# nmonette/TO-UED

Hardware: NVIDIA B200
Metric: gridworld agent env-steps/sec incl. LPG update (higher is better)
Workload: dtype f16/bf16 operands, f32 accumulate (GRU); f32 elsewhere

## Files before the change

include/toued.h:

```cpp
#ifndef TOUED_H
#define TOUED_H
#include <stdint.h>
#ifdef __cplusplus
extern "C" {
#endif

#define TOUED_LEVEL_BYTES 192

const char* toued_last_error(void);
int toued_version(void);

int toued_rollout(const void* levels, const uint32_t* keys, const float* actor,
                  const uint8_t* forced_actions, int32_t* state, int32_t* obs, uint8_t* action,
                  float* reward, uint8_t* done, float* ep_return, int n_agents, int n_workers,
                  int rollout_len, int obs_dim, int max_grid_size, int max_n_objs, int reset_first,
                  void* stream);

int toued_env_step(const void* levels, const uint32_t* keys, const int32_t* actions, int32_t* state,
                   int32_t* obs, float* reward, uint8_t* done, int n_agents, int n_workers,
                   int max_grid_size, int max_n_objs, void* stream);
int toued_env_reset(const void* levels, int32_t* state, int32_t* obs, int n_agents, int n_workers,
                    int max_grid_size, void* stream);


// ... 78 lines not shown
                    float lr_actor, float lr_critic, float max_grad_norm, float gamma, float gae_lambda,
                    float entropy_coeff, int outer_product_quirk, void* stream);

int toued_es_ask(const uint32_t* key, const float* mean, float sigma, float* candidates, int popsize,
                 int n_params, int cand_stride, void* stream);
int toued_es_tell(const float* candidates, const float* fitness, float* mean, float* m, float* v,
                  int popsize, int n_params, int cand_stride, float sigma, float lrate, float beta1,
                  float beta2, float eps, int gen_counter, float mean_decay, void* stream);

int toued_es_ask_shard(const uint32_t* key, const float* mean, float sigma, float* candidates, int popsize_global,
                       int n_params, int cand_stride, int pair_offset, int n_pairs, void* stream);
int toued_es_grad_partial(const float* candidates, const float* fitness, const float* mean, float* grad_sum,
                          int n_members, int n_params, int cand_stride, float sigma, void* stream);
int toued_es_adam(const float* grad_sum, float* mean, float* m, float* v, int popsize_global, int n_params,
                  float sigma, float lrate, float beta1, float beta2, float eps, int gen_counter, float mean_decay,
                  void* stream);

int toued_plr_reset_lowest(float* score, uint8_t* active, uint8_t* is_new, int buffer_size, int minimum_new,
                           int* reset_ids, void* stream);
int toued_plr_select(uint32_t key0, uint32_t key1, float* score, uint8_t* active, uint8_t* is_new, int buffer_size,
                     const int* old_ids, const uint8_t* terminated, const float* new_scores, int n_agents,
                     float p_replay, float temperature, int shuffle_rounds, int* new_ids, void* stream);

int toued_generate_levels_desc_bytes(void);
int toued_generate_levels(const void* gen_desc, const uint32_t* keys, const int32_t* buffer_ids, void* levels_out,
                          int32_t* lifetimes_out, int n_levels, void* stream);

int toued_optimal_return(const void* levels, int n_levels, int horizon, int max_grid_size, int max_n_objs,
                         double* out, void* stream);

int toued_get_nash(const float* game, const float* x0, const float* y0, float* x_out, float* y_out,
                   int n, int x_nz, int y_nz, int num_iters, float lr, void* stream);
int toued_projection_simplex(float* v, int n, int max_nz, void* stream);


int toued_init_tables(const uint32_t* keys, const uint8_t* mask, float* tables, int n_agents,
                      int obs_dim, int n_out, void* stream);
int toued_masked_reset(const void* levels, const uint8_t* mask, int32_t* state, int32_t* obs,
                       int32_t* step, int n_agents, int n_workers, int max_grid_size, void* stream);

int toued_host_iota_bits(const uint32_t* keys, int n_keys, int n, uint32_t* out);


int toued_key_split(const uint32_t* keys_in, int n_keys, int num, int offset, int count, uint32_t* out,
                    void* stream);
int toued_key_chain(const uint32_t* keys_in, int n_keys, int chain_len, uint32_t* keys_out,
                    uint32_t* carry_out, void* stream);


int toued_tc_gemm_test(const float* A, const float* B, void* scratch_img, float* D, void* stream);
int toued_tc_gemm_mixed_test(const float* A, const float* B, void* scratch_img, float* D, void* stream);
int toued_tc_gemm_mn_test(const float* A, const float* B, void* scratch_img, float* D, int lbo, int sbo,
                          int kadv, void* stream);
int toued_tc_gemm_mn2_test(const float* A, const float* B, void* scratch_img, float* D, void* stream);

int toued_pack_wh_forward(const float* lpg_params, void* wh_img, int lifetime_conditioning, void* stream);
int toued_gru_forward_tc(const float* x, const uint8_t* done, const float* lpg_params, const void* wh_img,
                         void* h16, void* fac, void* hpimg, float* pi_hat, float* y_hat, int n_agents,
                         int n_workers, int rollout_len, int lifetime_conditioning, void* stream);
int toued_pack_wh_forward_multi(const float* lpg_params, void* wh_img, int lifetime_conditioning, int n_sets,
                                int lpg_stride, void* stream);
int toued_gru_forward_tc_multi(const float* x, const uint8_t* done, const float* lpg_params, const void* wh_img,
                               float* pi_hat, float* y_hat, int n_agents, int n_workers, int rollout_len,
                               int lifetime_conditioning, int lpg_stride, void* stream);

int toued_pack_wh_backward(const float* lpg_params, void* whb_img, void* stream);
#define TOUED_STATUS_NONFINITE_COT 1u
#define TOUED_STATUS_FP16_RANGE 2u
int toued_cotangent_max(const float* d_pi_hat, const float* d_y_hat, int n_agents, int n_workers, int rollout_len,
                        uint32_t* cotangent_max, void* stream);
int toued_gru_backward_tc(const uint8_t* done, const float* lpg_params, const void* whb_img,
                          const void* h16, const void* fac, const float* y_hat, const float* d_pi_hat,
                          const float* d_y_hat, void* dgimg, float* dl, float* dx, uint32_t* cotangent_max,
                          int n_agents, int n_workers, int rollout_len, int lifetime_conditioning, void* stream);
int toued_wgrad_tc_splits(void);
int toued_wgrad_tc_small_splits(void);
int toued_lpg_wgrad_tc(const void* hpimg, const void* dgimg, const void* ximg, const void* h16,
                       const float* d_pi_hat, const float* dl, float* wh_partials, float* small_partials,
                       uint32_t* cotangent_max, int n_agents, int n_workers, int rollout_len, int accumulate,
                       void* stream);

#ifdef __cplusplus
}
#endif
#endif
```

to_ued_b200/_lib.py:

```python
from __future__ import annotations

import ctypes as C
import os

_HERE = os.path.dirname(os.path.abspath(__file__))
_VARIANT = os.environ.get("TOUED_LIB_VARIANT", "")
LIB_PATH = os.path.join(_HERE, f"libtoued_{_VARIANT}.so" if _VARIANT else "libtoued.so")

_lib = None


class TouedError(RuntimeError):
    pass


def lib() -> C.CDLL:
    global _lib
    if _lib is None:
        if not os.path.exists(LIB_PATH):
            raise TouedError(
                f"{LIB_PATH} is missing: the CUDA extension is not built. "
                "Run `python -m to_ued_b200.csrc.build` (there is no CPU fallback).")
        _lib = C.CDLL(LIB_PATH)
        _declare(_lib)
    return _lib


_P, _I, _F = C.c_void_p, C.c_int, C.c_float

SIGNATURES = {
    "toued_rollout": [_P] * 10 + [_I] * 7 + [_P],
    "toued_env_step": [_P] * 7 + [_I] * 4 + [_P],
    "toued_env_reset": [_P] * 3 + [_I] * 3 + [_P],
    "toued_sort_tokens": [_P] * 2 + [_I] * 3 + [_P],
    "toued_lpg_prepare": [_P] * 11 + [_I] * 6 + [_P],
    "toued_gru_forward": [_P] * 7 + [_I] * 5 + [_P],
    "toued_agent_update": [_P] * 12 + [_I] * 4 + [_F] * 4 + [_I, _P, _P],
    "toued_agent_scratch_floats": [_I] * 4,
    "toued_meta_loss": [_P] * 10 + [_I] * 5 + [_F] * 3 + [_I, _P],
    "toued_agent_backward": [_P] * 14 + [_I] * 4 + [_F] * 9 + [_P, _P],
    "toued_transpose_wh": [_P] * 3,
    "toued_gru_backward": [_P] * 10 + [_I] * 4 + [_P],
    "toued_lpg_wgrad_workspace_floats": [],
    "toued_lpg_wgrad": [_P] * 11 + [_I] * 6 + [_P],
    "toued_reduce_partials": [_P, _P, _I, _I, _I, _P],
    "toued_lpg_wgrad_splits": [_I],
    "toued_lpg_wgrad_workspace_offset": [_I],
    "toued_lpg_wgrad_embed": [_P] * 7 + [_I] * 6 + [_P],
    "toued_cotangent_max": [_P, _P, _I, _I, _I, _P, _P],
    "toued_pack_wh_backward": [_P] * 3,
    "toued_gru_backward_tc": [_P] * 12 + [_I] * 4 + [_P],
    "toued_wgrad_tc_splits": [],
    "toued_wgrad_tc_small_splits": [],
    "toued_lpg_wgrad_tc": [_P] * 9 + [_I] * 4 + [_P],
    "toued_adam": [_P] * 4 + [_I, _I] + [_F] * 4 + [_P],
    "toued_adam_dev": [_P] * 5 + [_I] + [_F] * 4 + [_P],
    "toued_sgd_clip": [_P] * 3 + [_I, _F, _F, _P],
    "toued_get_nash": [_P] * 5 + [_I] * 4 + [_F, _P],
    "toued_projection_simplex": [_P, _I, _I, _P],
    "toued_es_ask": [_P, _P, _F, _P, _I, _I, _I, _P],
    "toued_es_tell": [_P] * 5 + [_I, _I, _I] + [_F] * 5 + [_I, _F, _P],
    "toued_es_ask_shard": [_P, _P, _F, _P, _I, _I, _I, _I, _I, _P],
    "toued_es_grad_partial": [_P] * 4 + [_I, _I, _I, _F, _P],
    "toued_es_adam": [_P] * 4 + [_I, _I] + [_F] * 5 + [_I, _F, _P],
    "toued_a2c_update": [_P] * 12 + [_I] * 4 + [_F] * 6 + [_I, _P],
    "toued_a2c_train": [_P] * 15 + [_I] * 7 + [_F] * 6 + [_I, _P],
    "toued_init_tables": [_P] * 3 + [_I] * 3 + [_P],
    "toued_masked_reset": [_P] * 5 + [_I] * 3 + [_P],
    "toued_generate_levels_desc_bytes": [],
    "toued_generate_levels": [_P] * 5 + [_I, _P],
    "toued_plr_reset_lowest": [_P] * 3 + [_I, _I, _P, _P],
    "toued_plr_select": [C.c_uint32, C.c_uint32] + [_P] * 3 + [_I] + [_P] * 3 + [_I, _F, _F, _I, _P, _P],
    "toued_tc_gemm_test": [_P] * 5,
    "toued_tc_gemm_mixed_test": [_P] * 5,
    "toued_tc_gemm_mn_test": [_P] * 4 + [_I] * 3 + [_P],
    "toued_tc_gemm_mn2_test": [_P] * 5,
    "toued_pack_wh_forward": [_P, _P, _I, _P],
    "toued_pack_wh_forward_multi": [_P, _P, _I, _I, _I, _P],
    "toued_gru_forward_tc_multi": [_P] * 6 + [_I] * 5 + [_P],
    "toued_host_iota_bits": [_P, _I, _I, _P],
    "toued_key_split": [_P, _I, _I, _I, _I, _P, _P],
    "toued_key_chain": [_P, _I, _I, _P, _P, _P],
    "toued_gru_forward_tc": [_P] * 9 + [_I] * 4 + [_P],
    "toued_optimal_return": [_P] + [_I] * 4 + [_P, _P],
}


def _declare(l):
    l.toued_last_error.restype = C.c_char_p
    l.toued_last_error.argtypes = []
    l.toued_version.restype = _I
    l.toued_version.argtypes = []
    for name, args in SIGNATURES.items():
        fn = getattr(l, name)
        fn.restype = _I
        fn.argtypes = args


def ptr(t):
    if t is None:
        return None
    if not t.is_cuda:
        raise TouedError("to_ued_b200 ops need CUDA tensors (there is no CPU fallback)")
    if not t.is_contiguous():
        raise TouedError("to_ued_b200 ops need contiguous tensors")
    return t.data_ptr()


def stream_ptr():
    import torch
    return torch.cuda.current_stream().cuda_stream


KERNELS_PER_CALL = {"toued_adam_dev": 2, "toued_sgd_clip": 2, "toued_lpg_wgrad": 3, "toued_init_tables": 2, "toued_lpg_wgrad_tc": 2, "toued_pack_wh_forward": 2, "toued_pack_wh_forward_multi": 2}
LAUNCHES = {}
GRAPH_KERNELS = [0]
ENV_STEPS = [0]
PROFILE = None


H2D_BYTES = [0]


def h2d(t):
    H2D_BYTES[0] += int(t.numel() * t.element_size()) if hasattr(t, "element_size") else int(t.nbytes)
    return t


def reset_counters(profile=False):
# ... 34 lines not shown
```

to_ued_b200/csrc/gru_backward_tc.cu:

```cuda
#include "tc.cuh"
#include "lpg_common.cuh"
#include "../../include/toued.h"

constexpr int BT_M = 128;
constexpr int BT_THREADS = 11 * 32;
constexpr int BT_ACHUNK = BT_M * 128;
constexpr int BT_SSTAGE = 4 * BT_ACHUNK;
constexpr int BT_CSTAGE = 2 * BT_ACHUNK;
constexpr int BT_BSLICE = LPG_H * 32;
constexpr int BT_NSB = 6;
constexpr int BT_ICHUNK = 512;

__global__ void pack_wh_bwd_kernel(const float* __restrict__ Wh, __half* __restrict__ img) {
    const int i = blockIdx.x * blockDim.x + threadIdx.x;
    if (i >= LPG_H * LPG_G) return;
    const int j = i / LPG_G, c = i % LPG_G;
    char* base = reinterpret_cast<char*>(img) + (size_t)(c >> 4) * BT_BSLICE;
    *reinterpret_cast<__half*>(base + k16_offset(j, c & 15)) = __float2half_rn(Wh[i]);
}

extern "C" int toued_pack_wh_backward(const float* lpg_params, void* whb_img, void* stream) {
    pack_wh_bwd_kernel<<<(LPG_H * LPG_G + 255) / 256, 256, 0, (cudaStream_t)stream>>>(
        lpg_params + lpg_offsets(5).Wh, (__half*)whb_img);
    TOUED_LAUNCH_CHECK();
    return 0;
}

__device__ __forceinline__ uint4 ldg_stream(const __half* p) {
    uint4 r;
    asm volatile("ld.global.nc.L1::no_allocate.v4.u32 {%0, %1, %2, %3}, [%4];" : "=r"(r.x), "=r"(r.y), "=r"(r.z), "=r"(r.w) : "l"(p));
    return r;
}
__device__ __forceinline__ void unpack8h(const uint4& r, float (&v)[8]) {
    const __half2* h = reinterpret_cast<const __half2*>(&r);
#pragma unroll
    for (int e = 0; e < 4; ++e) { const float2 f = __half22float2(h[e]); v[2 * e] = f.x; v[2 * e + 1] = f.y; }
}
__global__ void __launch_bounds__(BT_THREADS, 1)
gru_backward_tc_kernel(const uint8_t* __restrict__ done, const float* __restrict__ lpg, int X,
                       const unsigned char* __restrict__ whb_img, const __half* __restrict__ h16,
                       const __half* __restrict__ fac, const float* __restrict__ y_hat,
                       const float* __restrict__ d_pi_hat, const float* __restrict__ d_y_hat,
                       unsigned char* __restrict__ dgimg, float* __restrict__ dl_out, float* __restrict__ dx,
                       uint32_t* __restrict__ cotmax, int R, int L, int W) {
    extern __shared__ __align__(1024) unsigned char smem_raw[];
    unsigned char* smem = smem_raw + ((1024u - (smem_u32(smem_raw) & 1023u)) & 1023u);
    unsigned char* sS = smem;
    unsigned char* sC = sS + 2 * BT_SSTAGE;
    unsigned char* sB = sC + BT_CSTAGE;
    unsigned char* sI = sB + BT_NSB * BT_BSLICE;
    float* swp = reinterpret_cast<float*>(sI + BT_ICHUNK);
    float* sWy = swp + LPG_H;
    float* sWi = sWy + LPG_H * LPG_Y;
    float* sWi2 = sWi + LPG_H * 4;
    float* sdx = sWi2 + LPG_H * 2;
    __shared__ __align__(8) uint64_t b_full[BT_NSB], b_empty[BT_NSB], k_full[4], k_empty[4], s_empty[2], q_full;
    __shared__ uint32_t tmem_base_s;

    const LpgOffsets o = lpg_offsets(X);
    const int tid = threadIdx.x, warp = tid >> 5, lane = tid & 31;
    const int row0 = blockIdx.x * BT_M;

    if (tid == 0) {
        for (int s = 0; s < BT_NSB; ++s) { mbar_init(&b_full[s], 1); mbar_init(&b_empty[s], 1); }
        for (int k = 0; k < 4; ++k) { mbar_init(&k_full[k], 4); mbar_init(&k_empty[k], 2); }
        mbar_init(&s_empty[0], 1); mbar_init(&s_empty[1], 1); mbar_init(&q_full, 1);
        mbar_fence_init();
    }
    if (warp == 9) tmem_alloc(&tmem_base_s, 512);
    for (int i = tid; i < LPG_H; i += BT_THREADS) swp[i] = lpg[o.w_pi + i];
    for (int i = tid; i < LPG_H * LPG_Y; i += BT_THREADS) sWy[i] = lpg[o.W_y + i];
    for (int i = tid; i < LPG_H * 6; i += BT_THREADS) {
        const int u = i / 6, q = i % 6;
        const float w = lpg[o.Wi + (3 + q / 3) * LPG_G + (q % 3) * LPG_H + u];
        if (q < 4) sWi[u * 4 + q] = w; else sWi2[u * 2 + q - 4] = w;
    }
    for (int i = tid; i < 16 * 16; i += BT_THREADS) {
        const int n = i >> 4, k = i & 15;
        *reinterpret_cast<__half*>(sI + k16_offset(n, k)) = __float2half_rn(n == k ? 1.0f : 0.0f);
    }
    fence_proxy_async_smem();
    tc_fence_before();
    __syncthreads();
    tc_fence_after();
    const uint32_t tmem_base = tmem_base_s;
    const size_t R32 = ((size_t)R + 31) >> 5;
    const size_t tstride = R32 * 32 * LPG_H;

    if (warp == 8) {
        if (lane == 0) {
            uint32_t it = 0;
            for (int t = 0; t < L; ++t) {
                if (t + 1 == L) break;
                for (int ub = 0; ub < 4; ++ub)
                    for (int kk = 0; kk < 4; ++kk) {
                        const int ks = ((kk & 1) << 1) | (kk >> 1);
                        for (int g = 0; g < 3; ++g, ++it) {
                            const int s = it % BT_NSB;
                            mbar_wait(&b_empty[s], ((it / BT_NSB) & 1) ^ 1);
                            mbar_expect_tx(&b_full[s], BT_BSLICE);
                            bulk_g2s(sB + s * BT_BSLICE, whb_img + (size_t)(g * 16 + ub * 4 + ks) * BT_BSLICE, BT_BSLICE, &b_full[s]);
                        }
                    }
            }
        }
    } else if (warp == 9) {
        {
            constexpr uint32_t idesc256 = tc_idesc(BT_M, 256, 0), idesc16 = tc_idesc(BT_M, 16, 0);
            const uint32_t s_addr = smem_u32(sS), c_addr = smem_u32(sC), i_addr = smem_u32(sI);
            const uint64_t cd0 = tc_smem_desc(c_addr), idd = tc_smem_desc_k16(i_addr);
            uint32_t it = 0;
            uint32_t ait = 0;
            for (int t = 0; t < L; ++t) {
                const uint32_t q_addr = tmem_base + (t & 1) * 256;
                const bool mma = t + 1 < L;
                for (int ub = 0; ub < 4; ++ub, ++ait) {
                    const uint64_t ad0 = tc_smem_desc(s_addr + (ait & 1) * BT_SSTAGE);
#pragma unroll
                    for (int kk = 0; kk < 4; ++kk) {
                        const int ks = ((kk & 1) << 1) | (kk >> 1);
                        uint32_t sg[3];
                        if (mma) {
#pragma unroll
                            for (int g = 0; g < 3; ++g, ++it) {
                                sg[g] = it % BT_NSB;
                                mbar_wait(&b_full[sg[g]], (it / BT_NSB) & 1);
                            }
                        }
                        mbar_wait(&k_full[ks], ait & 1);
                        tc_fence_after();
                        if (elect_one()) {
                            if (mma) {
#pragma unroll
                                for (int g = 0; g < 3; ++g)
                                    tc_mma(q_addr, ad0 + (uint64_t)((g * BT_ACHUNK) >> 4) + 2 * ks,
                                           tc_smem_desc_k16(smem_u32(sB + sg[g] * BT_BSLICE)), idesc256, (ub | kk | g) != 0);
                                tc_mma(q_addr + ub * 64 + ks * 16, cd0 + 2 * ks, idd, idesc16, 1u);
                                tc_mma(q_addr + ub * 64 + ks * 16, cd0 + (uint64_t)(BT_ACHUNK >> 4) + 2 * ks, idd, idesc16, 1u);
#pragma unroll
                                for (int g = 0; g < 3; ++g) tc_commit(&b_empty[sg[g]]);
                            }
                            tc_commit(&k_empty[ks]);
                            if (mma && ub == 3 && kk == 3) tc_commit(&q_full);
                        }
                        __syncwarp();
                    }
                }
            }
        }
    } else if (warp == 10) {
        if (lane == 0) {
            const uint32_t s_addr = smem_u32(sS);
            const size_t Rp = ((size_t)R + 63) & ~(size_t)63;
            const int nsub = ((size_t)row0 + 64 < Rp) ? 2 : 1;
            uint32_t ait = 0;
            for (int t = 0; t < L; ++t) {
                for (int ub = 0; ub < 4; ++ub, ++ait) {
#pragma unroll
                    for (int kk = 0; kk < 4; ++kk) {
                        const int ks = ((kk & 1) << 1) | (kk >> 1);
                        mbar_wait(&k_full[ks], ait & 1);
                        mbar_arrive(&k_empty[ks]);
                    }
                    const size_t itok0 = (size_t)t * Rp + row0;
                    const uint32_t src0 = s_addr + (ait & 1) * BT_SSTAGE;
#pragma unroll
                    for (int g = 0; g < 4; ++g)
                        for (int sub = 0; sub < nsub; ++sub)
                            bulk_s2g(dgimg + tile_img_offset(itok0 + sub * 64, 16, (g * 4 + ub) * 64), src0 + g * BT_ACHUNK + sub * 8192, 8192);
                    bulk_commit();
                    if (ait > 0) {
                        bulk_wait_read_1();
                        mbar_arrive(&s_empty[(ait - 1) & 1]);
                    }
                }
            }
            bulk_wait_read();
            mbar_arrive(&s_empty[(ait - 1) & 1]);
            bulk_wait_all();
        }
    } else {
        const int q = warp & 3, hf = warp >> 2;
        const int rl = q * 32 + lane;
        const int row = row0 + rl;
        const bool rv = row < R;
        const int rsafe = rv ? row : 0;
        const int n_ag = rsafe / W, w_ag = rsafe % W;
        uint32_t ait = 0;
        float range_max = 0.0f;
        const uint32_t sS_u32 = smem_u32(sS), sC_u32 = smem_u32(sC);
        const float S = cotmax ? cot_scale_from_max(*cotmax) : 1.0f;
        struct FacLoads { uint4 r, z, n, hn, hx; };
        const size_t fbase = rb32_index(0, R32, rsafe, hf * 32);
        const __half* p_r = fac + fac_index(0, R32, rsafe, hf * 32, 0);
        const __half* p_z = fac + fac_index(0, R32, rsafe, hf * 32, 1);
        const __half* p_n = fac + fac_index(0, R32, rsafe, hf * 32, 2);
        const __half* p_hn = fac + fac_index(0, R32, rsafe, hf * 32, 3);
        const __half* p_hx = h16 + fbase;
        const int tlast = L - 1;
        auto issue_fac = [&](int t_, int ub_, int c8_) {
            FacLoads l;
            const size_t off = (size_t)t_ * tstride + (size_t)((ub_ * 8 + c8_) << 8);
            const size_t foff = 4 * (size_t)t_ * tstride + (size_t)((ub_ * 8 + c8_) << 8);
            l.r = ldg_stream(p_r + foff);
            l.z = ldg_stream(p_z + foff);
            l.n = ldg_stream(p_n + foff);
            l.hn = ldg_stream(p_hn + foff);
            l.hx = ldg_stream(p_hx + off + (t_ < tlast ? tstride : 0));
            return l;
        };
        struct RowLoads { float4 y0, y1, d0, d1; float dpi; uint8_t dn, dn_hp; };
        auto issue_row = [&](int t_) {
            RowLoads r;
            const size_t tok_ = (size_t)t_ * R + rsafe;
            const float4* q0 = reinterpret_cast<const float4*>(y_hat + tok_ * 8);
            const float4* q1 = reinterpret_cast<const float4*>(d_y_hat + tok_ * 8);
            r.y0 = q0[0]; r.y1 = q0[1]; r.d0 = q1[0]; r.d1 = q1[1];
            r.dpi = d_pi_hat[tok_];
            r.dn = t_ > 0 ? done[((size_t)n_ag * L + (t_ - 1)) * W + w_ag] : (uint8_t)1;
            r.dn_hp = t_ + 1 < L ? done[((size_t)n_ag * L + t_) * W + w_ag] : (uint8_t)1;
            return r;
        };
        FacLoads nxt = issue_fac(0, 0, 0);
        RowLoads rnx = issue_row(0);
        for (int t = 0; t < L; ++t) {
            const size_t tok = (size_t)t * R + rsafe;
            float dl[8], dpi;
            const RowLoads rc = rnx;
            if (t + 1 < L) rnx = issue_row(t + 1);
            {
                const float yh[8] = {rc.y0.x, rc.y0.y, rc.y0.z, rc.y0.w, rc.y1.x, rc.y1.y, rc.y1.z, rc.y1.w};
                const float dy[8] = {rc.d0.x, rc.d0.y, rc.d0.z, rc.d0.w, rc.d1.x, rc.d1.y, rc.d1.z, rc.d1.w};
                float s = 0.f;
#pragma unroll
                for (int i = 0; i < 8; ++i) s = fmaf(yh[i], dy[i], s);
#pragma unroll
                for (int i = 0; i < 8; ++i) dl[i] = rv ? S * (yh[i] * (dy[i] - s)) : 0.0f;
                dpi = rv ? S * rc.dpi : 0.0f;
                if (hf == 0 && rv) {
                    float4* qo = reinterpret_cast<float4*>(dl_out + tok * 8);
                    qo[0] = make_float4(dl[0], dl[1], dl[2], dl[3]);
                    qo[1] = make_float4(dl[4], dl[5], dl[6], dl[7]);
                }
            }
            const float nd = (t > 0 && rv && !rc.dn) ? 1.0f : 0.0f;
            const float nd_hp = rc.dn_hp ? 0.0f : 1.0f;
            if (t > 0) { mbar_wait(&q_full, (t - 1) & 1); tc_fence_after(); }
            const uint32_t p_addr = tmem_base + ((t - 1) & 1) * 256 + ((uint32_t)(q * 32) << 16);
            float dx3 = 0.f, dx4 = 0.f;
            for (int ub = 0; ub < 4; ++ub) {
                const int ubase = ub * 64 + hf * 32;
                const uint32_t sSb = sS_u32 + (ait & 1) * BT_SSTAGE;
#pragma unroll
                for (int c8 = 0; c8 < 4; ++c8) {
                    const int u0 = ubase + c8 * 8;
                    float carry[8];
                    if (t > 0) tmem_ld8(p_addr + u0, carry);
                    const FacLoads cur = nxt;
                    {
                        int t2 = t, ub2 = ub, c2 = c8 + 1;
                        if (c2 == 4) { c2 = 0; ++ub2; if (ub2 == 4) { ub2 = 0; t2 = min(t + 1, tlast); } }
                        nxt = issue_fac(t2, ub2, c2);
                    }
                    if (t > 0) tmem_ld_wait();
                    else {
#pragma unroll
                        for (int e = 0; e < 8; ++e) carry[e] = 0.f;
                    }
                    float gr_[8], zz[8], gn_[8], hn_[8], hx[8];
                    const uint32_t zw[4] = {cur.z.x, cur.z.y, cur.z.z, cur.z.w};
                    unpack8h(cur.r, gr_); unpack8h(make_uint4(zw[0] & 0x7FFF7FFFu, zw[1] & 0x7FFF7FFFu, zw[2] & 0x7FFF7FFFu, zw[3] & 0x7FFF7FFFu), zz);
                    unpack8h(cur.n, gn_); unpack8h(cur.hn, hn_); unpack8h(cur.hx, hx);
                    float gr[8], gz[8], ghn[8], gan[8], cz[8];
#pragma unroll
                    for (int e = 0; e < 8; ++e) {
                        const int u = u0 + e;
                        float dh = nd * carry[e];
                        {
                            const float4 w0 = *reinterpret_cast<const float4*>(sWy + u * 8), w1 = *reinterpret_cast<const float4*>(sWy + u * 8 + 4);
                            float hd = dpi * swp[u];
                            hd = fmaf(dl[0], w0.x, hd); hd = fmaf(dl[1], w0.y, hd); hd = fmaf(dl[2], w0.z, hd); hd = fmaf(dl[3], w0.w, hd);
                            hd = fmaf(dl[4], w1.x, hd); hd = fmaf(dl[5], w1.y, hd); hd = fmaf(dl[6], w1.z, hd); hd = fmaf(dl[7], w1.w, hd);
                            dh += ((zw[e >> 1] >> (15 + 16 * (e & 1))) & 1u) ? 0.0f : hd;
                        }
                        if (!rv) dh = 0.0f;
                        const float omz = 1.0f - zz[e];
                        gan[e] = dh * omz * (1.0f - gn_[e] * gn_[e]);
                        ghn[e] = gan[e] * gr_[e];
                        gr[e] = ghn[e] * hn_[e] * (1.0f - gr_[e]);
                        gz[e] = dh * (nd_hp * hx[e] - gn_[e]) * zz[e] * omz;
                        cz[e] = dh * zz[e];
                        range_max = fmax3_nan(range_max, fabsf(dh), fabsf(gr[e]));
                        {
                            const float4 w0 = *reinterpret_cast<const float4*>(sWi + u * 4);
                            const float2 w1 = *reinterpret_cast<const float2*>(sWi2 + u * 2);
                            dx3 = fmaf(gr[e], w0.x, fmaf(gz[e], w0.y, fmaf(gan[e], w0.z, dx3)));
                            dx4 = fmaf(gr[e], w0.w, fmaf(gz[e], w1.x, fmaf(gan[e], w1.y, dx4)));
                        }
                    }
                    uint4 czh4, czl4;
                    {
                        uint32_t hi[4], lo[4];
#pragma unroll
                        for (int e2 = 0; e2 < 4; ++e2) {
                            hi[e2] = pack_h2_sat(cz[2 * e2], cz[2 * e2 + 1]);
                            const float2 f = __half22float2(*reinterpret_cast<const __half2*>(&hi[e2]));
                            lo[e2] = pack_h2_sat(cz[2 * e2] - f.x, cz[2 * e2 + 1] - f.y);
                        }
                        czh4 = make_uint4(hi[0], hi[1], hi[2], hi[3]);
                        czl4 = make_uint4(lo[0], lo[1], lo[2], lo[3]);
                    }
                    if (c8 == 0 && ait >= 2) mbar_wait(&s_empty[ait & 1], ((ait >> 1) & 1) ^ 1);
                    if ((c8 & 1) == 0 && ait > 0) mbar_wait(&k_empty[hf * 2 + (c8 >> 1)], (ait & 1) ^ 1);
                    const uint32_t so = sw128_offset(BT_M, rl, hf * 32 + c8 * 8);
                    st_shared_v4(sSb + so + 0 * BT_ACHUNK, pack8h_sat(gr));
                    st_shared_v4(sSb + so + 1 * BT_ACHUNK, pack8h_sat(gz));
                    st_shared_v4(sSb + so + 2 * BT_ACHUNK, pack8h_sat(ghn));
                    st_shared_v4(sSb + so + 3 * BT_ACHUNK, pack8h_sat(gan));
                    st_shared_v4(sC_u32 + so, czh4);
                    st_shared_v4(sC_u32 + so + BT_ACHUNK, czl4);
                    if (c8 & 1) {
                        fence_proxy_async_smem();
                        tc_fence_before();
                        __syncwarp();
                        if (lane == 0) mbar_arrive(&k_full[hf * 2 + (c8 >> 1)]);
                    }
                }
                ++ait;
            }
            if (hf > 0) { sdx[((hf - 1) * BT_M + rl) * 2] = dx3; sdx[((hf - 1) * BT_M + rl) * 2 + 1] = dx4; }
            asm volatile("bar.sync 1, 256;" ::: "memory");
            if (hf == 0 && rv) {
                dx3 += sdx[rl * 2]; dx4 += sdx[rl * 2 + 1];
                *reinterpret_cast<float2*>(dx + ((size_t)t * R + row) * 2) = make_float2(dx3, dx4);
            }
            asm volatile("bar.sync 1, 256;" ::: "memory");
        }
        if (__any_sync(0xffffffffu, !(range_max <= 65504.0f)) && lane == 0 && cotmax) atomicOr(cotmax + 1, TOUED_STATUS_FP16_RANGE);
    }
    tc_fence_before();
    __syncthreads();
    if (warp == 9) tmem_dealloc(tmem_base, 512);
}

static size_t gru_bwd_tc_smem() {
    return 2 * BT_SSTAGE + BT_CSTAGE + BT_NSB * BT_BSLICE + BT_ICHUNK + sizeof(float) * (LPG_H + LPG_H * LPG_Y + LPG_H * 6 + BT_M * 2) + 1024;
}

extern "C" int toued_gru_backward_tc(const uint8_t* done, const float* lpg_params, const void* whb_img,
                                     const void* h16, const void* fac, const float* y_hat, const float* d_pi_hat,
                                     const float* d_y_hat, void* dgimg, float* dl, float* dx, uint32_t* cotangent_max,
                                     int n_agents, int n_workers, int rollout_len, int lifetime_conditioning, void* stream) {
    const int R = n_agents * n_workers;
    TOUED_CHECK(R > 0 && rollout_len > 0, "toued_gru_backward_tc: empty problem");
    const size_t smem = gru_bwd_tc_smem();
    TOUED_CUDA(cudaFuncSetAttribute(gru_backward_tc_kernel, cudaFuncAttributeMaxDynamicSharedMemorySize, (int)smem));
    gru_backward_tc_kernel<<<(R + BT_M - 1) / BT_M, BT_THREADS, smem, (cudaStream_t)stream>>>(
        done, lpg_params, lifetime_conditioning ? 7 : 5, (const unsigned char*)whb_img, (const __half*)h16,
        (const __half*)fac, y_hat, d_pi_hat, d_y_hat, (unsigned char*)dgimg, dl, dx, cotangent_max, R, rollout_len, n_workers);
    TOUED_LAUNCH_CHECK();
    return 0;
}
```

to_ued_b200/csrc/tc.cuh:

```cuda
#pragma once
#include "common.cuh"
#include <cuda_fp16.h>
#include <cuda_bf16.h>

constexpr int TC_KB_ELEMS = 64;
constexpr int TC_UMMA_K = 16;

__host__ __device__ __forceinline__ uint32_t sw128_offset(int rows, int row, int k) {
    const int kb = k >> 6, kin = k & 63;
    const int chunk = kin >> 3;
    return (uint32_t)kb * (uint32_t)rows * 128u + (uint32_t)row * 128u + (uint32_t)((chunk ^ (row & 7)) << 4) +
           (uint32_t)((kin & 7) << 1);
}

__host__ __device__ __forceinline__ size_t tile_img_offset(size_t tok, int n_col_groups, int col) {
    const size_t tb = tok >> 6; const int r = (int)(tok & 63), cg = col >> 6, cin = col & 63;
    return ((tb * n_col_groups + cg) << 13) + (size_t)r * 128 + (size_t)(((cin >> 3) ^ (r & 7)) << 4) + (size_t)((cin & 7) << 1);
}

__host__ __device__ __forceinline__ size_t rb32_index(size_t t, size_t n_row_blocks, int row, int u) {
    return (((t * n_row_blocks + (size_t)(row >> 5)) * 32 + (size_t)(u >> 3)) << 8) + (size_t)((row & 31) << 3) + (size_t)(u & 7);
}

__host__ __device__ __forceinline__ size_t fac_index(size_t t, size_t n_row_blocks, int row, int u, int plane) {
    return ((((t * n_row_blocks + (size_t)(row >> 5)) * 4 + (size_t)plane) * 32 + (size_t)(u >> 3)) << 8) + (size_t)((row & 31) << 3) + (size_t)(u & 7);
}

__device__ __forceinline__ uint64_t tc_smem_desc(uint32_t smem_addr) {
    return (uint64_t)((smem_addr >> 4) & 0x3FFFu) | (1ull << 16) | (64ull << 32) | (1ull << 46) | (2ull << 61);
}
__host__ __device__ __forceinline__ uint32_t k16_offset(int row, int k) {
    return (uint32_t)(row >> 3) * 256u + (uint32_t)(k >> 3) * 128u + (uint32_t)(row & 7) * 16u + (uint32_t)(k & 7) * 2u;
}
__device__ __forceinline__ uint64_t tc_smem_desc_k16(uint32_t smem_addr) {
    return (uint64_t)((smem_addr >> 4) & 0x3FFFu) | ((uint64_t)(128u >> 4) << 16) | ((uint64_t)(256u >> 4) << 32) |
           (1ull << 46);
}
__device__ __forceinline__ uint64_t tc_smem_desc_mn(uint32_t smem_addr, uint32_t lbo_bytes) {
    return (uint64_t)((smem_addr >> 4) & 0x3FFFu) | ((uint64_t)((lbo_bytes >> 4) & 0x3FFFu) << 16) | (64ull << 32) |
           (1ull << 46) | (2ull << 61);
}
__device__ __forceinline__ uint64_t tc_smem_desc_mn_plain(uint32_t smem_addr, uint32_t lbo_bytes, uint32_t sbo_bytes) {
    return (uint64_t)((smem_addr >> 4) & 0x3FFFu) | ((uint64_t)((lbo_bytes >> 4) & 0x3FFFu) << 16) |
           ((uint64_t)((sbo_bytes >> 4) & 0x3FFFu) << 32) | (1ull << 46);
}
__host__ __device__ constexpr uint32_t tc_idesc_mn(int M, int N, int fmt) {
    return (1u << 4) | ((uint32_t)fmt << 7) | ((uint32_t)fmt << 10) | (1u << 15) | (1u << 16) |
           ((uint32_t)(N >> 3) << 17) | ((uint32_t)(M >> 4) << 24);
}
__host__ __device__ constexpr uint32_t tc_idesc(int M, int N, int fmt) {
    return (1u << 4) | ((uint32_t)fmt << 7) | ((uint32_t)fmt << 10) | ((uint32_t)(N >> 3) << 17) |
           ((uint32_t)(M >> 4) << 24);
}
__device__ __forceinline__ void tc_mma(uint32_t tmem_d, uint64_t adesc, uint64_t bdesc, uint32_t idesc, uint32_t accumulate) {
    asm volatile("{\n\t.reg .pred p;\n\tsetp.ne.b32 p, %4, 0;\n\t"
                 "tcgen05.mma.cta_group::1.kind::f16 [%0], %1, %2, %3, p;\n\t}\n"
                 ::"r"(tmem_d), "l"(adesc), "l"(bdesc), "r"(idesc), "r"(accumulate) : "memory");
}
__device__ __forceinline__ void tc_mma_ts(uint32_t tmem_d, uint32_t tmem_a, uint64_t bdesc, uint32_t idesc, uint32_t accumulate) {
    asm volatile("{\n\t.reg .pred p;\n\tsetp.ne.b32 p, %4, 0;\n\t"
                 "tcgen05.mma.cta_group::1.kind::f16 [%0], [%1], %2, %3, p;\n\t}\n"
                 ::"r"(tmem_d), "r"(tmem_a), "l"(bdesc), "r"(idesc), "r"(accumulate) : "memory");
}
__device__ __forceinline__ bool elect_one() {
    uint32_t pred;
    asm volatile("{\n\t.reg .pred p;\n\telect.sync _|p, 0xffffffff;\n\tselp.u32 %0, 1, 0, p;\n\t}" : "=r"(pred));
    return pred != 0;
}
__device__ __forceinline__ void tc_commit(uint64_t* bar) {
    asm volatile("tcgen05.commit.cta_group::1.mbarrier::arrive::one.shared::cluster.b64 [%0];" ::"r"(smem_u32(bar)) : "memory");
}
__device__ __forceinline__ void tc_fence_before() { asm volatile("tcgen05.fence::before_thread_sync;" ::: "memory"); }
__device__ __forceinline__ void tc_fence_after() { asm volatile("tcgen05.fence::after_thread_sync;" ::: "memory"); }
__device__ __forceinline__ void fence_proxy_async_smem() { asm volatile("fence.proxy.async.shared::cta;" ::: "memory"); }

__device__ __forceinline__ void tmem_alloc(uint32_t* smem_dst, uint32_t ncols) {
    asm volatile("tcgen05.alloc.cta_group::1.sync.aligned.shared::cta.b32 [%0], %1;" ::"r"(smem_u32(smem_dst)), "r"(ncols) : "memory");
    asm volatile("tcgen05.relinquish_alloc_permit.cta_group::1.sync.aligned;" ::: "memory");
}
__device__ __forceinline__ void tmem_dealloc(uint32_t taddr, uint32_t ncols) {
    asm volatile("tcgen05.dealloc.cta_group::1.sync.aligned.b32 %0, %1;" ::"r"(taddr), "r"(ncols) : "memory");
}
__device__ __forceinline__ void tmem_ld8(uint32_t taddr, float (&v)[8]) {
    uint32_t r[8];
    asm volatile("tcgen05.ld.sync.aligned.32x32b.x8.b32 {%0, %1, %2, %3, %4, %5, %6, %7}, [%8];"
                 : "=r"(r[0]), "=r"(r[1]), "=r"(r[2]), "=r"(r[3]), "=r"(r[4]), "=r"(r[5]), "=r"(r[6]), "=r"(r[7])
                 : "r"(taddr));
#pragma unroll
    for (int i = 0; i < 8; ++i) v[i] = __uint_as_float(r[i]);
}
__device__ __forceinline__ void tmem_st4(uint32_t taddr, const uint4& v) {
    asm volatile("tcgen05.st.sync.aligned.32x32b.x4.b32 [%0], {%1, %2, %3, %4};" ::"r"(taddr), "r"(v.x), "r"(v.y), "r"(v.z), "r"(v.w) : "memory");
}
__device__ __forceinline__ uint4 tmem_ld4(uint32_t taddr) {
    uint4 r;
    asm volatile("tcgen05.ld.sync.aligned.32x32b.x4.b32 {%0, %1, %2, %3}, [%4];"
                 : "=r"(r.x), "=r"(r.y), "=r"(r.z), "=r"(r.w) : "r"(taddr));
    return r;
}
__device__ __forceinline__ void tmem_st_wait() { asm volatile("tcgen05.wait::st.sync.aligned;" ::: "memory"); }
// ... 63 lines not shown
```

to_ued_b200/csrc/wgrad_tc.cu:

```cuda
#include "tc.cuh"
#include "lpg_common.cuh"
#include "../../include/toued.h"

constexpr int SMT_WI = 0, SMT_BHN = 8 * LPG_G, SMT_WPI = SMT_BHN + LPG_H, SMT_WY = SMT_WPI + LPG_H,
              SMT_BPI = SMT_WY + LPG_H * LPG_Y, SMT_BY = SMT_BPI + 1, SMT_TOTAL = SMT_BY + LPG_Y;
constexpr int WT_THREADS = 192;
constexpr int WT_NS = 3;
constexpr int WT_STAGE = 9 * 8192;

__global__ void __launch_bounds__(WT_THREADS, 1)
wgrad_wh_tc_kernel(const unsigned char* __restrict__ hpimg, const unsigned char* __restrict__ dgimg,
                   const unsigned char* __restrict__ ximg, float* __restrict__ partial, float* __restrict__ small_partial,
                   const uint32_t* __restrict__ cotmax, int n_tok_blocks, int blocks_per_split, int accumulate) {
    extern __shared__ __align__(1024) unsigned char smem_raw[];
    unsigned char* smem = smem_raw + ((1024u - (smem_u32(smem_raw) & 1023u)) & 1023u);
    __shared__ __align__(8) uint64_t full[WT_NS], empty[WT_NS], done_bar;
    __shared__ uint32_t tmem_base_s;
    const int tid = threadIdx.x, warp = tid >> 5, lane = tid & 31;
    const int type = blockIdx.x % 6, split = blockIdx.x / 6;
    const bool xt = type >= 4;
    const int jt = (type >> 1) & 1, ct = type & 1;
    const int tb0 = split * blocks_per_split;
    const int tb1 = min(n_tok_blocks, tb0 + blocks_per_split);
    const int nblk = max(0, tb1 - tb0);

    if (tid == 0) {
        for (int s = 0; s < WT_NS; ++s) { mbar_init(&full[s], 1); mbar_init(&empty[s], 1); }
        mbar_init(&done_bar, 1);
        mbar_fence_init();
    }
    if (warp == 5) tmem_alloc(&tmem_base_s, 512);
    tc_fence_before();
    __syncthreads();
    tc_fence_after();
    const uint32_t tmem_base = tmem_base_s;

    if (warp == 4) {
        if (lane == 0) {
            for (int i = 0; i < nblk; ++i) {
                const int s = i % WT_NS;
                mbar_wait(&empty[s], ((i / WT_NS) & 1) ^ 1);
                mbar_expect_tx(&full[s], xt ? 9 * 8192 : 8 * 8192);
                unsigned char* st = smem + s * WT_STAGE;
                const size_t tb = (size_t)(tb0 + i);
                if (!xt) {
                    bulk_g2s(st, hpimg + ((tb * 4 + 2 * jt) << 13), 2 * 8192, &full[s]);
                    bulk_g2s(st + 2 * 8192, dgimg + ((tb * 16 + 6 * ct) << 13), 6 * 8192, &full[s]);
                } else {
                    bulk_g2s(st, ximg + (tb << 13), 8192, &full[s]);
                    bulk_g2s(st + 8192, dgimg + ((tb * 16 + 8 * ct) << 13), 7 * 8192, &full[s]);
                    bulk_g2s(st + 8 * 8192, dgimg + ((tb * 16 + 8 * ct + 7) << 13), 8192, &full[s]);
                }
            }
        }
    } else if (warp == 5) {
        {
            constexpr uint32_t idesc = tc_idesc_mn(128, 192, 0), idesc_x = tc_idesc_mn(64, 256, 0);
            for (int i = 0; i < nblk; ++i) {
                const int s = i % WT_NS;
                mbar_wait(&full[s], (i / WT_NS) & 1);
                tc_fence_after();
                const uint32_t a0 = smem_u32(smem + s * WT_STAGE);
                if (elect_one()) {
                if (!xt) {
                    const uint32_t b0 = a0 + 2 * 8192;
#pragma unroll
                    for (int ks = 0; ks < 4; ++ks) {
                        const uint64_t ad = tc_smem_desc_mn(a0 + ks * 2048, 8192);
                        tc_mma(tmem_base, ad, tc_smem_desc_mn(b0 + ks * 2048, 8192), idesc, (i | ks) != 0);
                        tc_mma(tmem_base + 192, ad, tc_smem_desc_mn(b0 + 3 * 8192 + ks * 2048, 8192), idesc, (i | ks) != 0);
                    }
                } else {
                    const uint32_t b0 = a0 + 8192;
#pragma unroll
                    for (int ks = 0; ks < 4; ++ks) {
                        const uint64_t ad = tc_smem_desc_mn(a0 + ks * 2048, 0);
                        tc_mma(tmem_base, ad, tc_smem_desc_mn(b0 + ks * 2048, 8192), idesc_x, (i | ks) != 0);
                        tc_mma(tmem_base + 256, ad, tc_smem_desc_mn(b0 + 4 * 8192 + ks * 2048, 8192), idesc_x, (i | ks) != 0);
                    }
                }
                tc_commit(&empty[s]);
                }
                __syncwarp();
            }
            if (elect_one()) tc_commit(&done_bar);
            __syncwarp();
        }
    } else {
        mbar_wait(&done_bar, 0);
        tc_fence_after();
        const float inv_s = cotmax ? 1.0f / cot_scale_from_max(*cotmax) : 1.0f;
        if (xt) {
            if (warp == 0) {
                float* out = small_partial + (size_t)split * SMT_TOTAL;
                auto dst_of = [&](int cc) {
                    if (ct == 0) return SMT_WI + lane * LPG_G + cc;
                    if (cc >= 256) return SMT_WI + lane * LPG_G + 512 + (cc - 256);
                    return lane == 7 ? SMT_BHN + cc : -1;
                };
                for (int c = 0; c < 512; c += 32) {
                    float v[4][8], o[4][8];
#pragma unroll
                    for (int i = 0; i < 4; ++i) {
                        if (nblk > 0) tmem_ld8(tmem_base + c + 8 * i, v[i]);
                        else {
#pragma unroll
                            for (int e = 0; e < 8; ++e) v[i][e] = 0.f;
                        }
                    }
                    if (nblk > 0) tmem_ld_wait();
                    if (lane < 8) {
#pragma unroll
                        for (int i = 0; i < 4; ++i)
#pragma unroll
                            for (int e = 0; e < 8; ++e) { const int d = dst_of(c + 8 * i + e); o[i][e] = d >= 0 ? out[d] : 0.0f; }
#pragma unroll
                        for (int i = 0; i < 4; ++i)
#pragma unroll
                            for (int e = 0; e < 8; ++e) { const int d = dst_of(c + 8 * i + e); if (d >= 0) out[d] = fmaf(v[i][e], inv_s, o[i][e]); }
                    }
                }
            }
        } else {
        const int j = jt * 128 + warp * 32 + lane;
        float* out = partial + (size_t)split * LPG_H * LPG_G + (size_t)j * LPG_G + ct * 384;
        for (int c = 0; c < 384; c += 64) {
            float4 pre[16];
            float4* p = reinterpret_cast<float4*>(out + c);
            if (accumulate) {
#pragma unroll
                for (int i = 0; i < 16; ++i) pre[i] = p[i];
// ... 327 lines not shown
```

Baseline: 470.5 million.

## Write GRU backward gate grads directly as K-major global image, drop TMA store warp

The GRU backward kernel now transposes packed gate-gradient fragments in registers (movmatrix plus shuffles) and streams them straight to global memory in a K-major tiled image. This replaces the dedicated bulk-store warp and the double-buffered shared staging. The wgrad kernel's B operand descriptors switch from MN-major to K-major to match the new layout. The change frees shared memory and a warp, and removes the s_empty synchronization. In exchange, the compute warps take on extra shuffle and transpose work plus uncoalesced-pattern global stores.

New measurement: 445.4 million, median of 6. 0.947x the previous value.

```diff
diff --git a/include/toued.h b/include/toued.h
--- a/include/toued.h
+++ b/include/toued.h
@@ -154,6 +154,7 @@
 int toued_tc_gemm_mixed_test(const float* A, const float* B, void* scratch_img, float* D, void* stream);
 int toued_tc_gemm_mn_test(const float* A, const float* B, void* scratch_img, float* D, int lbo, int sbo,
                           int kadv, void* stream);
+int toued_tc_gemm_mn_k_test(const float* A, const float* B, void* scratch_img, float* D, void* stream);
 int toued_tc_gemm_mn2_test(const float* A, const float* B, void* scratch_img, float* D, void* stream);
 
 int toued_pack_wh_forward(const float* lpg_params, void* wh_img, int lifetime_conditioning, void* stream);
diff --git a/to_ued_b200/_lib.py b/to_ued_b200/_lib.py
--- a/to_ued_b200/_lib.py
+++ b/to_ued_b200/_lib.py
@@ -75,6 +75,7 @@
     "toued_tc_gemm_mixed_test": [_P] * 5,
     "toued_tc_gemm_mn_test": [_P] * 4 + [_I] * 3 + [_P],
     "toued_tc_gemm_mn2_test": [_P] * 5,
+    "toued_tc_gemm_mn_k_test": [_P] * 5,
     "toued_pack_wh_forward": [_P, _P, _I, _P],
     "toued_pack_wh_forward_multi": [_P, _P, _I, _I, _I, _P],
     "toued_gru_forward_tc_multi": [_P] * 6 + [_I] * 5 + [_P],
diff --git a/to_ued_b200/csrc/gru_backward_tc.cu b/to_ued_b200/csrc/gru_backward_tc.cu
--- a/to_ued_b200/csrc/gru_backward_tc.cu
+++ b/to_ued_b200/csrc/gru_backward_tc.cu
@@ -3,9 +3,9 @@
 #include "../../include/toued.h"
 
 constexpr int BT_M = 128;
-constexpr int BT_THREADS = 11 * 32;
+constexpr int BT_THREADS = 10 * 32;
 constexpr int BT_ACHUNK = BT_M * 128;
-constexpr int BT_SSTAGE = 4 * BT_ACHUNK;
+constexpr int BT_SSTAGE = 3 * BT_ACHUNK;
 constexpr int BT_CSTAGE = 2 * BT_ACHUNK;
 constexpr int BT_BSLICE = LPG_H * 32;
 constexpr int BT_NSB = 6;
@@ -30,6 +30,26 @@
     uint4 r;
     asm volatile("ld.global.nc.L1::no_allocate.v4.u32 {%0, %1, %2, %3}, [%4];" : "=r"(r.x), "=r"(r.y), "=r"(r.z), "=r"(r.w) : "l"(p));
     return r;
+}
+__device__ __forceinline__ uint32_t movmatrix_trans(uint32_t a) {
+    uint32_t d;
+    asm("movmatrix.sync.aligned.m8n8.trans.b16 %0, %1;" : "=r"(d) : "r"(a));
+    return d;
+}
+__device__ __forceinline__ uint4 transpose_tokens(const uint4& w, bool s0, bool s1) {
+    uint32_t y0 = movmatrix_trans(w.x), y1 = movmatrix_trans(w.y), y2 = movmatrix_trans(w.z), y3 = movmatrix_trans(w.w);
+    {
+        const uint32_t r0 = __shfl_xor_sync(0xffffffffu, s0 ? y0 : y1, 8), r1 = __shfl_xor_sync(0xffffffffu, s0 ? y2 : y3, 8);
+        if (s0) { y0 = r0; y2 = r1; } else { y1 = r0; y3 = r1; }
+    }
+    {
+        const uint32_t r0 = __shfl_xor_sync(0xffffffffu, s1 ? y0 : y2, 16), r1 = __shfl_xor_sync(0xffffffffu, s1 ? y1 : y3, 16);
+        if (s1) { y0 = r0; y1 = r1; } else { y2 = r0; y3 = r1; }
+    }
+    return make_uint4(__byte_perm(y0, y1, 0x5410), __byte_perm(y2, y3, 0x5410), __byte_perm(y0, y1, 0x7632), __byte_perm(y2, y3, 0x7632));
+}
+__device__ __forceinline__ void stg_stream(unsigned char* p, const uint4& v) {
+    asm volatile("st.global.L1::no_allocate.v4.b32 [%0], {%1, %2, %3, %4};" ::"l"(p), "r"(v.x), "r"(v.y), "r"(v.z), "r"(v.w) : "memory");
 }
 __device__ __forceinline__ void unpack8h(const uint4& r, float (&v)[8]) {
     const __half2* h = reinterpret_cast<const __half2*>(&r);
@@ -46,7 +66,7 @@
     extern __shared__ __align__(1024) unsigned char smem_raw[];
     unsigned char* smem = smem_raw + ((1024u - (smem_u32(smem_raw) & 1023u)) & 1023u);
     unsigned char* sS = smem;
-    unsigned char* sC = sS + 2 * BT_SSTAGE;
+    unsigned char* sC = sS + BT_SSTAGE;
     unsigned char* sB = sC + BT_CSTAGE;
     unsigned char* sI = sB + BT_NSB * BT_BSLICE;
     float* swp = reinterpret_cast<float*>(sI + BT_ICHUNK);
@@ -54,7 +74,7 @@
     float* sWi = sWy + LPG_H * LPG_Y;
     float* sWi2 = sWi + LPG_H * 4;
     float* sdx = sWi2 + LPG_H * 2;
-    __shared__ __align__(8) uint64_t b_full[BT_NSB], b_empty[BT_NSB], k_full[4], k_empty[4], s_empty[2], q_full;
+    __shared__ __align__(8) uint64_t b_full[BT_NSB], b_empty[BT_NSB], k_full[4], k_empty[4], q_full;
     __shared__ uint32_t tmem_base_s;
 
     const LpgOffsets o = lpg_offsets(X);
@@ -63,8 +83,8 @@
 
     if (tid == 0) {
         for (int s = 0; s < BT_NSB; ++s) { mbar_init(&b_full[s], 1); mbar_init(&b_empty[s], 1); }
-        for (int k = 0; k < 4; ++k) { mbar_init(&k_full[k], 4); mbar_init(&k_empty[k], 2); }
-        mbar_init(&s_empty[0], 1); mbar_init(&s_empty[1], 1); mbar_init(&q_full, 1);
+        for (int k = 0; k < 4; ++k) { mbar_init(&k_full[k], 4); mbar_init(&k_empty[k], 1); }
+        mbar_init(&q_full, 1);
         mbar_fence_init();
     }
     if (warp == 9) tmem_alloc(&tmem_base_s, 512);
@@ -109,13 +129,13 @@
             constexpr uint32_t idesc256 = tc_idesc(BT_M, 256, 0), idesc16 = tc_idesc(BT_M, 16, 0);
             const uint32_t s_addr = smem_u32(sS), c_addr = smem_u32(sC), i_addr = smem_u32(sI);
             const uint64_t cd0 = tc_smem_desc(c_addr), idd = tc_smem_desc_k16(i_addr);
+            const uint64_t ad0 = tc_smem_desc(s_addr);
             uint32_t it = 0;
             uint32_t ait = 0;
             for (int t = 0; t < L; ++t) {
                 const uint32_t q_addr = tmem_base + (t & 1) * 256;
                 const bool mma = t + 1 < L;
                 for (int ub = 0; ub < 4; ++ub, ++ait) {
-                    const uint64_t ad0 = tc_smem_desc(s_addr + (ait & 1) * BT_SSTAGE);
 #pragma unroll
                     for (int kk = 0; kk < 4; ++kk) {
                         const int ks = ((kk & 1) << 1) | (kk >> 1);
@@ -147,37 +167,6 @@
                     }
                 }
             }
-        }
-    } else if (warp == 10) {
-        if (lane == 0) {
-            const uint32_t s_addr = smem_u32(sS);
-            const size_t Rp = ((size_t)R + 63) & ~(size_t)63;
-            const int nsub = ((size_t)row0 + 64 < Rp) ? 2 : 1;
-            uint32_t ait = 0;
-            for (int t = 0; t < L; ++t) {
-                for (int ub = 0; ub < 4; ++ub, ++ait) {
-#pragma unroll
-                    for (int kk = 0; kk < 4; ++kk) {
-                        const int ks = ((kk & 1) << 1) | (kk >> 1);
-                        mbar_wait(&k_full[ks], ait & 1);
-                        mbar_arrive(&k_empty[ks]);
-                    }
-                    const size_t itok0 = (size_t)t * Rp + row0;
-                    const uint32_t src0 = s_addr + (ait & 1) * BT_SSTAGE;
-#pragma unroll
-                    for (int g = 0; g < 4; ++g)
-                        for (int sub = 0; sub < nsub; ++sub)
-                            bulk_s2g(dgimg + tile_img_offset(itok0 + sub * 64, 16, (g * 4 + ub) * 64), src0 + g * BT_ACHUNK + sub * 8192, 8192);
-                    bulk_commit();
-                    if (ait > 0) {
-                        bulk_wait_read_1();
-                        mbar_arrive(&s_empty[(ait - 1) & 1]);
-                    }
-                }
-            }
-            bulk_wait_read();
-            mbar_arrive(&s_empty[(ait - 1) & 1]);
-            bulk_wait_all();
         }
     } else {
         const int q = warp & 3, hf = warp >> 2;
@@ -188,7 +177,12 @@
         const int n_ag = rsafe / W, w_ag = rsafe % W;
         uint32_t ait = 0;
         float range_max = 0.0f;
-        const uint32_t sS_u32 = smem_u32(sS), sC_u32 = smem_u32(sC);
+        const uint32_t sSb = smem_u32(sS), sC_u32 = smem_u32(sC);
+        const size_t Rp = ((size_t)R + 63) & ~(size_t)63;
+        const bool img_ok = (size_t)row0 + q * 32 < Rp;
+        const bool ts0 = (lane >> 3) & 1, ts1 = (lane >> 4) & 1;
+        const int icol = hf * 32 + (lane >> 3) * 2 + ((lane >> 2) & 1);
+        unsigned char* const img0 = dgimg + (size_t)icol * 128 + (size_t)((((q & 1) * 4 + (lane & 3)) ^ (icol & 7)) << 4);
         const float S = cotmax ? cot_scale_from_max(*cotmax) : 1.0f;
         struct FacLoads { uint4 r, z, n, hn, hx; };
         const size_t fbase = rb32_index(0, R32, rsafe, hf * 32);
@@ -225,6 +219,7 @@
         RowLoads rnx = issue_row(0);
         for (int t = 0; t < L; ++t) {
             const size_t tok = (size_t)t * R + rsafe;
+            unsigned char* const img = img0 + ((((size_t)t * Rp + row0 + q * 32) >> 6) * 16 << 13);
             float dl[8], dpi;
             const RowLoads rc = rnx;
             if (t + 1 < L) rnx = issue_row(t + 1);
@@ -250,7 +245,6 @@
             float dx3 = 0.f, dx4 = 0.f;
             for (int ub = 0; ub < 4; ++ub) {
                 const int ubase = ub * 64 + hf * 32;
-                const uint32_t sSb = sS_u32 + (ait & 1) * BT_SSTAGE;
 #pragma unroll
                 for (int c8 = 0; c8 < 4; ++c8) {
                     const int u0 = ubase + c8 * 8;
@@ -310,13 +304,12 @@
                         czh4 = make_uint4(hi[0], hi[1], hi[2], hi[3]);
                         czl4 = make_uint4(lo[0], lo[1], lo[2], lo[3]);
                     }
-                    if (c8 == 0 && ait >= 2) mbar_wait(&s_empty[ait & 1], ((ait >> 1) & 1) ^ 1);
+                    const uint4 pr = pack8h_sat(gr), pz = pack8h_sat(gz), phn = pack8h_sat(ghn), pan = pack8h_sat(gan);
                     if ((c8 & 1) == 0 && ait > 0) mbar_wait(&k_empty[hf * 2 + (c8 >> 1)], (ait & 1) ^ 1);
                     const uint32_t so = sw128_offset(BT_M, rl, hf * 32 + c8 * 8);
-                    st_shared_v4(sSb + so + 0 * BT_ACHUNK, pack8h_sat(gr));
-                    st_shared_v4(sSb + so + 1 * BT_ACHUNK, pack8h_sat(gz));
-                    st_shared_v4(sSb + so + 2 * BT_ACHUNK, pack8h_sat(ghn));
-                    st_shared_v4(sSb + so + 3 * BT_ACHUNK, pack8h_sat(gan));
+                    st_shared_v4(sSb + so + 0 * BT_ACHUNK, pr);
+                    st_shared_v4(sSb + so + 1 * BT_ACHUNK, pz);
+                    st_shared_v4(sSb + so + 2 * BT_ACHUNK, phn);
                     st_shared_v4(sC_u32 + so, czh4);
                     st_shared_v4(sC_u32 + so + BT_ACHUNK, czl4);
                     if (c8 & 1) {
@@ -325,6 +318,13 @@
                         __syncwarp();
                         if (lane == 0) mbar_arrive(&k_full[hf * 2 + (c8 >> 1)]);
                     }
+                    if (img_ok) {
+                        unsigned char* d = img + ((size_t)ub << 13) + c8 * 1024;
+                        stg_stream(d, transpose_tokens(pr, ts0, ts1));
+                        stg_stream(d + 4 * 8192, transpose_tokens(pz, ts0, ts1));
+                        stg_stream(d + 8 * 8192, transpose_tokens(phn, ts0, ts1));
+                        stg_stream(d + 12 * 8192, transpose_tokens(pan, ts0, ts1));
+                    }
                 }
                 ++ait;
             }
@@ -344,7 +344,7 @@
 }
 
 static size_t gru_bwd_tc_smem() {
-    return 2 * BT_SSTAGE + BT_CSTAGE + BT_NSB * BT_BSLICE + BT_ICHUNK + sizeof(float) * (LPG_H + LPG_H * LPG_Y + LPG_H * 6 + BT_M * 2) + 1024;
+    return BT_SSTAGE + BT_CSTAGE + BT_NSB * BT_BSLICE + BT_ICHUNK + sizeof(float) * (LPG_H + LPG_H * LPG_Y + LPG_H * 6 + BT_M * 2) + 1024;
 }
 
 extern "C" int toued_gru_backward_tc(const uint8_t* done, const float* lpg_params, const void* whb_img,
diff --git a/to_ued_b200/csrc/tc.cuh b/to_ued_b200/csrc/tc.cuh
--- a/to_ued_b200/csrc/tc.cuh
+++ b/to_ued_b200/csrc/tc.cuh
@@ -16,6 +16,10 @@
 __host__ __device__ __forceinline__ size_t tile_img_offset(size_t tok, int n_col_groups, int col) {
     const size_t tb = tok >> 6; const int r = (int)(tok & 63), cg = col >> 6, cin = col & 63;
     return ((tb * n_col_groups + cg) << 13) + (size_t)r * 128 + (size_t)(((cin >> 3) ^ (r & 7)) << 4) + (size_t)((cin & 7) << 1);
+}
+__host__ __device__ __forceinline__ size_t tile_img_kmajor_offset(size_t tok, int n_col_groups, int col) {
+    const size_t tb = tok >> 6; const int r = (int)(tok & 63), cg = col >> 6, cin = col & 63;
+    return ((tb * n_col_groups + cg) << 13) + (size_t)cin * 128 + (size_t)(((r >> 3) ^ (cin & 7)) << 4) + (size_t)((r & 7) << 1);
 }
 
 __host__ __device__ __forceinline__ size_t rb32_index(size_t t, size_t n_row_blocks, int row, int u) {
@@ -46,6 +50,10 @@
 }
 __host__ __device__ constexpr uint32_t tc_idesc_mn(int M, int N, int fmt) {
     return (1u << 4) | ((uint32_t)fmt << 7) | ((uint32_t)fmt << 10) | (1u << 15) | (1u << 16) |
+           ((uint32_t)(N >> 3) << 17) | ((uint32_t)(M >> 4) << 24);
+}
+__host__ __device__ constexpr uint32_t tc_idesc_mn_k(int M, int N, int fmt) {
+    return (1u << 4) | ((uint32_t)fmt << 7) | ((uint32_t)fmt << 10) | (1u << 15) |
            ((uint32_t)(N >> 3) << 17) | ((uint32_t)(M >> 4) << 24);
 }
 __host__ __device__ constexpr uint32_t tc_idesc(int M, int N, int fmt) {
diff --git a/to_ued_b200/csrc/wgrad_tc.cu b/to_ued_b200/csrc/wgrad_tc.cu
--- a/to_ued_b200/csrc/wgrad_tc.cu
+++ b/to_ued_b200/csrc/wgrad_tc.cu
@@ -55,7 +55,7 @@
         }
     } else if (warp == 5) {
         {
-            constexpr uint32_t idesc = tc_idesc_mn(128, 192, 0), idesc_x = tc_idesc_mn(64, 256, 0);
+            constexpr uint32_t idesc = tc_idesc_mn_k(128, 192, 0), idesc_x = tc_idesc_mn_k(64, 256, 0);
             for (int i = 0; i < nblk; ++i) {
                 const int s = i % WT_NS;
                 mbar_wait(&full[s], (i / WT_NS) & 1);
@@ -67,16 +67,16 @@
 #pragma unroll
                     for (int ks = 0; ks < 4; ++ks) {
                         const uint64_t ad = tc_smem_desc_mn(a0 + ks * 2048, 8192);
-                        tc_mma(tmem_base, ad, tc_smem_desc_mn(b0 + ks * 2048, 8192), idesc, (i | ks) != 0);
-                        tc_mma(tmem_base + 192, ad, tc_smem_desc_mn(b0 + 3 * 8192 + ks * 2048, 8192), idesc, (i | ks) != 0);
+                        tc_mma(tmem_base, ad, tc_smem_desc(b0 + ks * 32), idesc, (i | ks) != 0);
+                        tc_mma(tmem_base + 192, ad, tc_smem_desc(b0 + 3 * 8192 + ks * 32), idesc, (i | ks) != 0);
                     }
                 } else {
                     const uint32_t b0 = a0 + 8192;
 #pragma unroll
                     for (int ks = 0; ks < 4; ++ks) {
                         const uint64_t ad = tc_smem_desc_mn(a0 + ks * 2048, 0);
-                        tc_mma(tmem_base, ad, tc_smem_desc_mn(b0 + ks * 2048, 8192), idesc_x, (i | ks) != 0);
-                        tc_mma(tmem_base + 256, ad, tc_smem_desc_mn(b0 + 4 * 8192 + ks * 2048, 8192), idesc_x, (i | ks) != 0);
+                        tc_mma(tmem_base, ad, tc_smem_desc(b0 + ks * 32), idesc_x, (i | ks) != 0);
+                        tc_mma(tmem_base + 256, ad, tc_smem_desc(b0 + 4 * 8192 + ks * 32), idesc_x, (i | ks) != 0);
                     }
                 }
                 tc_commit(&empty[s]);
```
